# Xiaohao-Liu/EliMRec

Hardware: AMD Instinct MI355X
Metric: BPR triplets/sec (Tiktok-shape, d=128x3) (higher is better)
Workload: dtype f32; 1 GPU; tiktok-shape-synthetic; num_items=76085, train_interactions=571503, recdim=64, layer_num=3, batch_per_gpu=2048, global_batch=2048, parallelism=colshard1, graph_table=column-sharded (64 of 64 columns per rank): hops need no communication, feature_tables=replicated S_m / c, feature_dtype=f32, columns_per_gpu=64, propagation=folded, head_rows=batch, step_issue=one host call per step (csrc/program.hip): 1243 of the 1243 timed steps

## Files before the change

elimrec_amd/_lib.py:

```python
import ctypes
import os

_HERE = os.path.dirname(os.path.abspath(__file__))
LIB_PATH = os.path.join(_HERE, "lib", "libelimrec_hip.so")

c_i32, c_i64, c_f32, c_u32, c_u64 = ctypes.c_int, ctypes.c_int64, ctypes.c_float, ctypes.c_uint32, ctypes.c_uint64
c_ptr, c_size = ctypes.c_void_p, ctypes.c_size_t

class CsrSplit(ctypes.Structure):
    _fields_ = [("long_threshold", ctypes.c_int32), ("n_long", ctypes.c_int32), ("n_seg", ctypes.c_int32),
                ("d_long_rows", ctypes.c_void_p), ("d_long_seg_ptr", ctypes.c_void_p),
                ("d_seg_bounds", ctypes.c_void_p), ("d_partials", ctypes.c_void_p), ("d_seg_row", ctypes.c_void_p),
                ("d_row_order", ctypes.c_void_p), ("d_tickets", ctypes.c_void_p), ("d_row_items", ctypes.c_void_p),
                ("n_row_items", ctypes.c_int32)]


class CsrDesc(ctypes.Structure):
    _fields_ = [("n_rows", ctypes.c_int64), ("d_rowptr", ctypes.c_void_p), ("d_col", ctypes.c_void_p),
                ("d_val", ctypes.c_void_p), ("split", CsrSplit)]


class LinearDesc(ctypes.Structure):
    _fields_ = [("d_A", ctypes.c_void_p), ("lda", ctypes.c_int64), ("d_W", ctypes.c_void_p), ("ldw", ctypes.c_int64),
                ("d_bias", ctypes.c_void_p), ("d_C", ctypes.c_void_p), ("ldc", ctypes.c_int64), ("M", ctypes.c_int64),
# ... 144 lines not shown
                                 c_ptr]),
    "elimrec_topk_reference_order": (c_i32, [c_ptr, c_i64, c_i64, c_i64, c_i32, c_ptr]),
    "elimrec_topk_reference_order_device": (c_i32, [c_ptr, c_i64, c_i64, c_i64, c_i32, c_ptr, c_ptr, c_ptr]),
    "elimrec_score_topk_ordered": (c_i32, [c_ptr, c_i64, c_i64, c_i64, c_ptr, c_i32, c_i32, c_i32, c_u32, c_i32, c_i32,
                                           c_ptr, c_ptr, c_ptr, c_ptr, c_i64, c_i32, c_ptr, c_ptr, c_ptr, c_size, c_i32, c_ptr]),
    "elimrec_plan_workspace": (c_size, [c_i64, c_i64, c_i64]),
    "elimrec_plan_tile_count": (c_i64, [c_i64, c_i64, c_i64, c_i64, c_i32]),
    "elimrec_plan_rows": (c_i32, [c_ptr, c_i64, c_i32, c_i32, c_i32, c_i32, c_i32, c_i64, c_i64, c_ptr, c_ptr, c_ptr, c_ptr, c_ptr, c_ptr, c_size, c_ptr]),
    "elimrec_plan_tiles": (c_i32, [c_ptr, c_i64, c_i32, c_i32, c_i32, c_i32, c_i32, c_i64, c_i64, c_ptr, c_ptr, c_ptr, c_i64, c_i64, c_i64, c_i64, c_i64,
                                   c_i64, c_ptr, c_ptr, c_ptr, c_ptr, c_ptr, c_ptr, c_ptr, c_ptr, c_size, c_ptr]),
    "elimrec_plan_scatter": (c_i32, [c_i64, c_i32, c_ptr, c_ptr, c_ptr, c_ptr, c_ptr, c_ptr, c_ptr, c_ptr, c_ptr]),
    "elimrec_slab_sweep_lds_rows": (c_size, [c_i32]),
    "elimrec_slab_sweep_hop": (c_i32, [c_ptr, c_ptr, c_i64, c_i64, c_ptr, c_i32, c_i32, c_i32, c_i32, c_i32, c_i32,
                                       c_ptr, c_ptr, c_ptr, c_ptr, c_f32, c_ptr]),
    "elimrec_slab_sweep_hop_adam": (c_i32, [c_ptr, c_ptr, c_i64, c_i64, c_ptr, c_i32, c_i32, c_i32, c_i32, c_i32, c_i32,
                                            c_ptr, c_ptr, c_ptr, c_ptr, c_f32, c_ptr, c_ptr, c_ptr, c_ptr, c_f32, c_f32, c_f32, c_f32, c_f32,
                                            c_i64, c_ptr]),
    "elimrec_slab_hop_bwd_w": (c_i32, [c_sell, c_i32, c_i32, c_i32, c_ptr, c_ptr, c_ptr, c_ptr, c_ptr, c_f32, c_ptr, c_size, c_i32,
                                       ctypes.POINTER(LinearBwdDesc), c_i32, c_ptr, c_size, c_i32, c_ptr]),
    "elimrec_slab_source_bits": (c_i32, [c_sell, c_i32, c_i32, c_i32, c_ptr, c_ptr, c_size, c_ptr]),
    "elimrec_slab_hop_adam": (c_i32, [c_sell, c_i32, c_i32, c_i32, c_ptr, c_ptr, c_ptr, c_ptr, c_f32, c_ptr, c_size, c_ptr, c_ptr,
                                      c_ptr, c_ptr, c_f32, c_f32, c_f32, c_f32, c_f32, c_i64, ctypes.POINTER(AdamJob), c_i32, c_ptr, c_i64,
                                      c_ptr, c_ptr]),
    "elimrec_slab_rows": (c_i32, [c_sell, c_i32, c_i32, c_i32, c_i64, ctypes.POINTER(c_ptr), c_ptr, c_ptr, c_ptr, c_i64, c_i32,
                                  c_ptr, c_i64, c_ptr, c_i64, c_i32, c_ptr]),
    "elimrec_slab_from_rows": (c_i32, [c_ptr, c_i64, c_i64, c_i64, c_i32, c_i32, c_ptr, c_ptr]),
    "elimrec_slab_to_rows": (c_i32, [c_ptr, c_i64, c_i32, c_i32, c_ptr, c_i64, c_i64, c_ptr]),
    "elimrec_slab_merge_rows": (c_i32, [c_ptr, c_ptr, c_i32, c_i64, c_i64, c_i64, c_i32, c_i32, c_i32, c_ptr, c_ptr, c_ptr, c_ptr]),
    "elimrec_adam_step_out": (c_i32, [c_ptr, c_ptr, c_ptr, c_ptr, c_ptr, c_i64, c_f32, c_f32, c_f32, c_f32, c_f32, c_i64,
                                      c_ptr]),
    "elimrec_head_pack_floats": (c_size, [c_i32, ctypes.POINTER(c_i32)]),
    "elimrec_head_pack_bwd_offset": (c_size, [c_i32, ctypes.POINTER(c_i32)]),
    "elimrec_head_fwd_fused": (c_i32, [c_ptr, c_ptr, c_i64, c_ptr, c_i64, c_ptr, c_i64, c_ptr, c_i32, ctypes.POINTER(c_ptr),
                                       ctypes.POINTER(c_i64), ctypes.POINTER(c_i32), ctypes.POINTER(c_ptr), ctypes.POINTER(c_ptr),
                                       c_ptr, c_ptr, c_ptr, c_ptr, ctypes.POINTER(c_ptr), ctypes.POINTER(c_ptr), c_ptr, c_size,
                                       c_ptr, c_i64, c_ptr, c_i64, c_i32, c_i32, c_ptr]),
    "elimrec_head_fwd_fused_peers": (c_i32, [c_ptr, c_ptr, c_i64, c_ptr, c_i32, c_i64, c_ptr, c_i32, ctypes.POINTER(c_ptr),
                                             ctypes.POINTER(c_i64), ctypes.POINTER(c_i32), ctypes.POINTER(c_ptr), ctypes.POINTER(c_ptr),
                                             c_ptr, c_ptr, c_ptr, c_ptr, ctypes.POINTER(c_ptr), ctypes.POINTER(c_ptr), c_ptr, c_size,
                                             c_ptr, c_i64, c_ptr, c_i64, c_i32, c_i32, c_ptr]),
    "elimrec_head_fwd_fused_rows": (c_i32, [ctypes.POINTER(HeadRows), c_ptr, c_ptr, c_i64, c_ptr, c_i32, ctypes.POINTER(c_ptr),
                                            ctypes.POINTER(c_i64), ctypes.POINTER(c_i32), ctypes.POINTER(c_ptr), ctypes.POINTER(c_ptr),
                                            c_ptr, c_ptr, c_ptr, c_ptr, ctypes.POINTER(c_ptr), ctypes.POINTER(c_ptr), c_ptr, c_size,
                                            c_ptr, c_i64, c_ptr, c_i64, c_i32, c_ptr]),
    "elimrec_head_fwd_fused_src16": (c_i32, [ctypes.POINTER(HeadSrc16), c_ptr, c_ptr, c_i64, c_ptr, c_i64, c_ptr, c_i64, c_i32,
                                             ctypes.POINTER(c_i32), ctypes.POINTER(c_ptr), ctypes.POINTER(c_ptr), c_ptr, c_ptr, c_ptr, c_ptr,
# ... 114 lines not shown
```

elimrec_amd/csrc/program.hip:

```cpp
#include "common.h"
#include <dlfcn.h>
#include <cstring>
#include <string>
#include <utility>
#include <vector>

namespace elimrec {

template <typename T> struct Unpack {
    static T get(uint64_t v) {
        if constexpr (std::is_pointer<T>::value) return reinterpret_cast<T>(static_cast<uintptr_t>(v));
        else if constexpr (std::is_same<T, float>::value) { uint32_t b = (uint32_t)v; float f; memcpy(&f, &b, 4); return f; }
        else return static_cast<T>(v);
    }
};
template <typename R, typename... A, size_t... I>
static R call_packed_impl(R (*f)(A...), const uint64_t *a, std::index_sequence<I...>) { return f(Unpack<A>::get(a[I])...); }
template <typename R, typename... A> static R call_packed(R (*f)(A...), const uint64_t *a) {
    static_assert(sizeof...(A) <= ELIMREC_PROGRAM_MAX_ARGS, "too many arguments for a program op");
    return call_packed_impl(f, a, std::index_sequence_for<A...>{});
}
template <typename R, typename... A> constexpr int arg_count(R (*)(A...)) { return (int)sizeof...(A); }

static unsigned event_flags(bool has_collectives) {
    return has_collectives ? hipEventDisableTiming : (hipEventDisableTiming | hipEventDisableSystemFence);
}

struct FnEntry { const char *name; int (*thunk)(const uint64_t *); int n_args; };
#define ELIMREC_FN(fn) {#fn, [](const uint64_t *a) -> int { return call_packed(fn, a); }, arg_count(fn)}
static const FnEntry kFns[] = {
    ELIMREC_FN(elimrec_batch_plan), ELIMREC_FN(elimrec_slab_hop), ELIMREC_FN(elimrec_slab_sweep_hop), ELIMREC_FN(elimrec_slab_sweep_hop_adam), ELIMREC_FN(elimrec_slab_source_bits), ELIMREC_FN(elimrec_slab_hop_bwd_w),
    ELIMREC_FN(elimrec_slab_hop_adam), ELIMREC_FN(elimrec_slab_rows), ELIMREC_FN(elimrec_slab_merge_rows),
    ELIMREC_FN(elimrec_head_fwd_fused), ELIMREC_FN(elimrec_bpr_head_rows),
    ELIMREC_FN(elimrec_bpr_head_rows_sum), ELIMREC_FN(elimrec_bpr_head_rows_sum_pub), ELIMREC_FN(elimrec_sum), ELIMREC_FN(elimrec_segment_apply_head_bwd),
    ELIMREC_FN(elimrec_segment_apply_head_bwd_packed), ELIMREC_FN(elimrec_segment_apply_head_bwd_sources),
    ELIMREC_FN(elimrec_segment_apply_head_bwd_split), ELIMREC_FN(elimrec_linear_fwd_batched), ELIMREC_FN(elimrec_linear_bwd_w_batched),
    ELIMREC_FN(elimrec_linear_bwd_w_batched_merge), ELIMREC_FN(elimrec_linear_bwd_w_reduce), ELIMREC_FN(elimrec_adam_multi),
    ELIMREC_FN(elimrec_source_rows_split), ELIMREC_FN(elimrec_copy_cols), ELIMREC_FN(elimrec_lookup_pack), ELIMREC_FN(elimrec_lookup_unpack),
    ELIMREC_FN(elimrec_lookup_counts), ELIMREC_FN(elimrec_adam_step_out),
    ELIMREC_FN(elimrec_peer_cols_to_rows), ELIMREC_FN(elimrec_rows_bitmap), ELIMREC_FN(elimrec_comm_all_gather), ELIMREC_FN(elimrec_comm_all_reduce_f32),
    ELIMREC_FN(elimrec_comm_all_to_all), ELIMREC_FN(elimrec_comm_all_to_all_v), ELIMREC_FN(elimrec_wide_from_master),
    ELIMREC_FN(elimrec_wide_rows), ELIMREC_FN(elimrec_wide_grad), ELIMREC_FN(elimrec_head_fwd_fused_rows), ELIMREC_FN(elimrec_head_fwd_fused_src16),
    ELIMREC_FN(elimrec_head_fwd_fused_peers),
};
constexpr int kNumFns = (int)(sizeof(kFns) / sizeof(kFns[0]));

typedef struct ncclComm *ncclComm_t;
struct NcclId { char internal[128]; };
struct Rccl {
    void *h = nullptr;
    int (*GetUniqueId)(NcclId *) = nullptr;
    int (*CommInitRank)(ncclComm_t *, int, NcclId, int) = nullptr;
    int (*CommDestroy)(ncclComm_t) = nullptr;
    int (*CommCount)(ncclComm_t, int *) = nullptr;
    int (*AllGather)(const void *, void *, size_t, int, ncclComm_t, hipStream_t) = nullptr;
// ... 185 lines not shown
```

elimrec_amd/csrc/slab.hip:

```cpp
#include "common.h"
#include "merge_rows.h"
#include "rows_args.h"
#include "bwd_w.h"
#include <cstdlib>

namespace elimrec {


struct SellArgs {
    const int32_t *item_dst, *item_len, *blk_off, *col;
    const float *val;
    int64_t n_rows, n_src;
    int n_seg, n_long;
    int item_begin, item_end;
    int seg_limit;
    int w4, w4_shift, gs, spg;
    const float4 *Xin;
    const uint32_t *src_mask;
    float4 *Xout;
    const float4 *Add;
    const uint32_t *add_mask;
    float scale;
    float4 *partials;
    const int32_t *long_rows, *long_seg_ptr;
// ... 329 lines not shown
    int64_t n;
    float step_size, inv_sqrt_bc2;
    int first_block;
};
struct AdamJobs {
    AdamJob j[8]; int n; int blocks;
    const float *sum_src; float *sum_dst; int sum_n;
};

__device__ __forceinline__ void fixed_order_sum_body(const float *__restrict__ x, int n, float *__restrict__ out, float *s) {
    for (int vt = threadIdx.x; vt < 1024; vt += 256) {
        float acc = 0.f;
        for (int i = vt; i < n; i += 1024) acc += x[i];
        s[vt] = acc;
    }
    __syncthreads();
    for (int w = 512; w > 0; w >>= 1) {
        for (int idx = threadIdx.x; idx < w; idx += 256) s[idx] += s[idx + w];
        __syncthreads();
    }
    if (threadIdx.x == 0) out[0] = s[0];
}

__device__ __forceinline__ void adam_jobs_body(const AdamJobs &jobs, int block, float beta1, float beta2, float eps, float wd) {
    int k = 0;
    while (k + 1 < jobs.n && block >= jobs.j[k + 1].first_block) ++k;
    const AdamJob &jb = jobs.j[k];
    const int nb = (k + 1 < jobs.n ? jobs.j[k + 1].first_block : jobs.blocks) - jb.first_block;
    for (int64_t i = (int64_t)(block - jb.first_block) * 256 + threadIdx.x; i < jb.n; i += (int64_t)nb * 256) {
        const float pi = jb.p_in[i];
        if (jb.copy_dst) jb.copy_dst[i] = pi;
        if (!jb.g) continue;
        const float gi = fmaf(wd, pi, jb.g[i]);
        const float mi = jb.m[i] + (1.f - beta1) * (gi - jb.m[i]);
        const float vi = fmaf(1.f - beta2, gi * gi, beta2 * jb.v[i]);
        const float denom = sqrtf(vi) * jb.inv_sqrt_bc2 + eps;
        jb.m[i] = mi;
        jb.v[i] = vi;
        const float po = pi - jb.step_size * (mi / denom);
        jb.p_out[i] = po;
    }
}

__global__ __launch_bounds__(256) void adam_multi_kernel(AdamJobs jobs, float beta1, float beta2, float eps, float wd) {
    adam_jobs_body(jobs, (int)blockIdx.x, beta1, beta2, eps, wd);
}

struct TierArgs {
    StreamArgs s;
    const int64_t *tile_off;
    const int32_t *tile_len, *tile_dst, *tile_long, *tcol, *long_index;
    const float *tval;
    int n_w4;
    int t1_base, tseg_base, tfin_base, n_tiles;
    int n_tiles_run;
    const uint64_t *ballots;
// ... 243 lines not shown
    }
}

#ifndef ELIMREC_TILE_WAVES
#define ELIMREC_TILE_WAVES 5
#endif
template <int LPR, int VPL, bool IN_BF16, bool OUT_BF16, bool MASKED>
__global__ __launch_bounds__(256, ELIMREC_TILE_WAVES) void sell_tier_kernel(TierArgs t) {
    tier_body<LPR, VPL, IN_BF16, OUT_BF16, MASKED, false>(t);
}

template <int LPR>
__global__ __launch_bounds__(256) void sell_tier_adam_kernel(TierArgs t, AdamJobs tail, int tail_block0) {
    __shared__ float scratch[4 * 64 * 8];
    if ((int)blockIdx.x >= tail_block0) {
        const int b = (int)blockIdx.x - tail_block0;
        if (b < tail.blocks) adam_jobs_body(tail, b, t.s.ad_beta1, t.s.ad_beta2, t.s.ad_eps, t.s.ad_wd);
        else fixed_order_sum_body(tail.sum_src, tail.sum_n, tail.sum_dst, scratch);
        return;
    }
    tier_body<LPR, 4, false, false, false, true, true>(t, scratch);
}

template <int LPR, bool MASKED>
__global__ __launch_bounds__(256, (LPR <= 8 ? 5 : 1)) void sell_tier_bwdw_kernel(TierArgs t, BwdBatch batch, int tail_block0, int tail_mode, int gx) {
    __shared__ float As[2][TRB * TN1];
    __shared__ float Bs[2][TRB * TN2];
    static_assert(2 * TRB * TN1 >= 4 * 64 * 8, "the hop's LDS scratch must fit the A stages");
    const int front = tail_block0 < 0 ? (-tail_block0 + 7) & ~7 : 0;
    if (tail_block0 < 0 ? (int)blockIdx.x < front : (int)blockIdx.x >= tail_block0) {
        const int b = tail_block0 < 0 ? (int)blockIdx.x : (int)blockIdx.x - tail_block0;
        if (tail_block0 < 0 && b >= -tail_block0) return;
        if (tail_mode == 1) { reduce_slabs_body(batch, b % gx, b / gx); return; }
        bwd_w_partial_body(batch, b, As, Bs);
        return;
    }
    tier_body<LPR, 4, false, false, MASKED, false, true>(t, &As[0][0], (unsigned)front);
}

static int log2_pow2(int x) {
    int s = 0;
    while ((1 << s) < x) ++s;
    return (1 << s) == x ? s : -1;
}

}

using namespace elimrec;

static size_t slab_partial_floats_bytes(const elimrec_sell *A, int ns, int w) {
    return align_up((size_t)(A->n_seg > 0 ? A->n_seg : 1) * ns * w * sizeof(float), 256);
}
static size_t slab_ticket_bytes(const elimrec_sell *A) { return align_up((size_t)8 * (A->n_long > 0 ? A->n_long : 1) * sizeof(int32_t), 256); }
static size_t slab_ballot_bytes(const elimrec_sell *A) {
    if (!A->tiered) return 0;
    const size_t tiles = (size_t)A->n_t4 + A->n_t1 + A->n_tseg + A->n_tfin;
    return align_up(tiles * (size_t)(A->tile_kmax > 0 ? A->tile_kmax : 1) * sizeof(uint64_t), 256);
}

extern "C" size_t elimrec_slab_partials_bytes(const elimrec_sell *A, int ns, int w) {
    if (!A || ns <= 0 || w <= 0) return 0;
    return slab_partial_floats_bytes(A, ns, w) + slab_ticket_bytes(A) + slab_ballot_bytes(A);
}

struct AdamEpilogue {
    const float *p_in; float *p_out, *m, *v;
    float step_size, inv_sqrt_bc2, beta1, beta2, eps, wd;
    int keep_grad;
    const AdamJobs *tail;
};

static int launch_tier(const elimrec_sell *A, int ns, int wl, int wl_shift, int gs, int spg, int lpr, const void *Xin,
                       const uint32_t *src_mask, void *Xout, const float *add,
                       const uint32_t *add_mask, float scale, float *partials, int flags, hipStream_t s,
                       const AdamEpilogue *adam = nullptr, const BwdBatch *bwdw = nullptr, int tail_mode = 0, int tail_blocks = 0,
                       int reduce_gx = 1) {
    const int seg_only = flags & 1;
    const bool bits_ready = (flags & 2) != 0;
    if (A->tile_groups != 64 / lpr) {
        set_error("slab_hop: the plan's wave tiles were laid out for %d lane groups per wave, this table geometry has %d",
                  A->tile_groups, 64 / lpr);
        return ELIMREC_E_BADARG;
    }
    ELIMREC_REQUIRE(A->d_tile_off && A->d_tile_len && A->d_tile_dst && A->d_tile_col && A->d_tile_val && A->n_t4 == 4 * A->n_w4 &&
                        A->n_t1 % 4 == 0 && A->n_tseg % 4 == 0 && A->n_tfin % 4 == 0 && (A->n_tseg == 0 || A->d_tile_long),
                    "slab_hop: bad tile plan");
    TierArgs t = {};
    StreamArgs &a = t.s;
    a.n_rows = A->n_rows; a.n_src = A->n_src; a.n_seg = A->n_seg; a.n_long = A->n_long;
    a.wl = wl; a.wl_shift = wl_shift; a.gs = gs; a.spg = spg;
    a.Xin = Xin; a.src_mask = src_mask; a.Xout = Xout;
    a.Add = seg_only ? nullptr : (const float4 *)add; a.add_mask = add_mask; a.scale = seg_only ? 1.0f : scale;
// ... 16 lines not shown
    int tail_block0 = (int)(per_group * gs);
    {
        if (bwdw && tail_blocks > 0 && !adam && tail_mode == 2) {
            tail_block0 = -tail_blocks;
            tail_blocks = (tail_blocks + 7) & ~7;
        }
    }
    AdamJobs tail = {};
    if (adam && adam->tail && (adam->tail->n > 0 || adam->tail->sum_src)) tail = *adam->tail;
    if (tail.n <= 0) tail.blocks = 0;
    const dim3 grid((unsigned)(per_group * gs)), grid_adam((unsigned)(per_group * gs) + (unsigned)tail.blocks + (tail.sum_src ? 1u : 0u));
    const bool masked = src_mask != nullptr;
    if (masked) {
        ELIMREC_REQUIRE(A->tile_kmax > 0, "slab_hop: bad tile plan (tile_kmax)");
        t.kmax = A->tile_kmax;
        uint64_t *ballots = (uint64_t *)((char *)a.tickets + slab_ticket_bytes(A));
        t.ballots = ballots;
        if (!bits_ready)
        hipLaunchKernelGGL(tile_ballot_kernel, dim3((unsigned)per_group, (unsigned)t.kmax), dim3(256), 0, s, t.tile_off, t.tcol, src_mask, 64 / lpr,
                           t.n_tiles_run, t.kmax, ballots);
    }
#define ELIMREC_TIER(LPR)                                                                                                     \
    do {                                                                                                                      \
        if (adam) hipLaunchKernelGGL((sell_tier_adam_kernel<LPR>), grid_adam, dim3(256), 0, s, t, tail, tail_block0);         \
        else if (bwdw && masked)                                                                                              \
            hipLaunchKernelGGL((sell_tier_bwdw_kernel<LPR, true>), dim3(grid.x + (unsigned)tail_blocks), dim3(256), 0, s, t,  \
                               *bwdw, tail_block0, tail_mode, reduce_gx);                                                     \
        else if (bwdw)                                                                                                        \
            hipLaunchKernelGGL((sell_tier_bwdw_kernel<LPR, false>), dim3(grid.x + (unsigned)tail_blocks), dim3(256), 0, s, t, \
                               *bwdw, tail_block0, tail_mode, reduce_gx);                                                     \
        else if (masked) hipLaunchKernelGGL((sell_tier_kernel<LPR, 4, false, false, true>), grid, dim3(256), 0, s, t);        \
        else hipLaunchKernelGGL((sell_tier_kernel<LPR, 4, false, false, false>), grid, dim3(256), 0, s, t);                   \
    } while (0)
    switch (lpr) {
        case 1: ELIMREC_TIER(1); break;
        case 2: ELIMREC_TIER(2); break;
        case 4: ELIMREC_TIER(4); break;
        case 8: ELIMREC_TIER(8); break;
        case 16: ELIMREC_TIER(16); break;
        case 32: ELIMREC_TIER(32); break;
        default: ELIMREC_TIER(64); break;
    }
#undef ELIMREC_TIER
    return check_hip(hipGetLastError(), "slab_hop(tiered)");
}

static int slab_geometry(const char *who, int ns, int w, int gs, int &w4_shift, int &spg, int &lpr) {
// ... 127 lines not shown
extern "C" int elimrec_slab_hop_bwd_w(const elimrec_sell *A, int ns, int w, int gs, const float *d_Xin, const uint32_t *d_src_mask,
                                      float *d_Xout, const float *d_add, const uint32_t *d_add_mask, float scale, float *d_partials,
                                      size_t partials_bytes, int flags, const elimrec_linear_bwd_desc *descs, int n,
                                      void *d_workspace, size_t workspace_bytes, int phase, void *stream) {
    ELIMREC_REQUIRE(A && d_Xin && d_Xout && d_Xin != d_Xout, "slab_hop_bwd_w: null pointer / alias");
    ELIMREC_REQUIRE(A->tiered && !(flags & 1), "slab_hop_bwd_w: needs a tiered (wave-tile) plan and a full hop");
    ELIMREC_REQUIRE(phase == 0 || phase == 1, "slab_hop_bwd_w: phase 0 (partial launch) or 1 (slab reduce)");
    ELIMREC_REQUIRE(descs && n >= 1 && n <= kMaxBatch, "slab_hop_bwd_w: 1..%d problems", kMaxBatch);
    ELIMREC_REQUIRE(d_workspace && workspace_bytes >= bwd_w_batched_bytes(descs, n), "slab_hop_bwd_w: weight-gradient workspace");
    int w4_shift, spg, lpr, rc;
    if ((rc = slab_geometry("slab_hop_bwd_w", ns, w, gs, w4_shift, spg, lpr))) return rc;
    if (!d_partials || partials_bytes < elimrec_slab_partials_bytes(A, ns, w)) {
        set_error("slab_hop_bwd_w: partial-row scratch too small");
        return ELIMREC_E_WORKSPACE;
    }
    BwdBatch batch;
    int blocks = 0, max_out = 0;
    if ((rc = bwd_w_build_batch(descs, n, d_workspace, batch, blocks, max_out))) return rc;
    const int gx = (4 * max_out + 255) / 256;
    return launch_tier(A, ns, w / 4, w4_shift, gs, spg, lpr, d_Xin, d_src_mask, d_Xout, d_add, d_add_mask, scale,
                       d_partials, flags, (hipStream_t)stream, nullptr, &batch, phase == 0 ? 2 : 1, phase == 0 ? blocks : gx * n, gx);
}

extern "C" int elimrec_slab_hop_adam(const elimrec_sell *A, int ns, int w, int gs, const float *d_Xin, float *d_grad_out,
                                     const float *d_add, const uint32_t *d_add_mask, float scale, float *d_partials,
                                     size_t partials_bytes, const float *d_p_in, float *d_p_out, float *d_m, float *d_v, float lr,
                                     float beta1, float beta2, float eps, float weight_decay, int64_t step,
                                     const elimrec_adam_job *tail_jobs, int n_tail_jobs, const float *d_sum_src, int64_t sum_n,
                                     float *d_sum_dst, void *stream) {
    ELIMREC_REQUIRE(A && d_Xin && d_p_in && d_p_out && d_m && d_v, "slab_hop_adam: null pointer");
    ELIMREC_REQUIRE(!d_sum_src || (d_sum_dst && sum_n >= 0 && sum_n < INT32_MAX), "slab_hop_adam: the sum needs a destination");
    ELIMREC_REQUIRE(A->tiered, "slab_hop_adam: needs a tiered (wave-tile) plan");
    ELIMREC_REQUIRE(step >= 1, "slab_hop_adam: 1-based step");
    ELIMREC_REQUIRE((const void *)d_Xin != (const void *)d_p_out && (const void *)d_Xin != (const void *)d_m &&
                        (const void *)d_Xin != (const void *)d_v, "slab_hop_adam: the gathered table must not be written");
    int w4_shift, spg, lpr, rc;
    if ((rc = slab_geometry("slab_hop_adam", ns, w, gs, w4_shift, spg, lpr))) return rc;
    if (!d_partials || partials_bytes < elimrec_slab_partials_bytes(A, ns, w)) {
        set_error("slab_hop_adam: partial-row scratch too small");
        return ELIMREC_E_WORKSPACE;
    }
    AdamEpilogue ad;
    ad.p_in = d_p_in; ad.p_out = d_p_out; ad.m = d_m; ad.v = d_v;
    const double bc1 = 1.0 - pow((double)beta1, (double)step), bc2 = 1.0 - pow((double)beta2, (double)step);
    ad.step_size = (float)((double)lr / bc1);
    ad.inv_sqrt_bc2 = (float)(1.0 / sqrt(bc2));
    ad.beta1 = beta1; ad.beta2 = beta2; ad.eps = eps; ad.wd = weight_decay; ad.keep_grad = d_grad_out ? 1 : 0;
    AdamJobs tail = {};
    ad.tail = nullptr;
    if (tail_jobs && n_tail_jobs > 0) {
        ELIMREC_REQUIRE(n_tail_jobs <= 8, "slab_hop_adam: at most 8 tail jobs");
        if ((rc = build_adam_jobs("slab_hop_adam", tail_jobs, n_tail_jobs, lr, beta1, beta2, tail))) return rc;
        ad.tail = &tail;
    }
    if (d_sum_src) { tail.sum_src = d_sum_src; tail.sum_dst = d_sum_dst; tail.sum_n = (int)sum_n; ad.tail = &tail; }
    return launch_tier(A, ns, w / 4, w4_shift, gs, spg, lpr, d_Xin, nullptr, d_grad_out, d_add, d_add_mask, scale,
                       d_partials, 0, (hipStream_t)stream, &ad);
}

extern "C" int elimrec_slab_rows(const elimrec_sell *A, int ns, int w, int L, int64_t U, const float *const *layers,
                                 const float *d_long, const int32_t *d_rows, const int32_t *d_counts, int64_t R,
                                 int n_lists, float *d_out0, int64_t ld_out0, float *d_narrow, int64_t ld_narrow,
                                 int narrow_by_node, void *stream) {
    ELIMREC_REQUIRE(A && layers && d_out0 && d_narrow, "slab_rows: null pointer");
    ELIMREC_REQUIRE(ld_out0 % 4 == 0 && ld_narrow % 4 == 0, "slab_rows: leading dimensions must be multiples of 4");
    ELIMREC_REQUIRE(n_lists >= 1 && (d_rows || n_lists == 1), "slab_rows: several lists need row ids");
    RowsArgs a = {};
    int rc;
    if ((rc = rows_args_fill("slab_rows", A, ns, w, L, U, layers, d_long, a))) return rc;
    a.rows = d_rows; a.counts = d_counts; a.R = R; a.n_lists = n_lists;
    a.out0 = d_out0; a.ld_out0 = ld_out0; a.narrow = d_narrow; a.ld_narrow = ld_narrow; a.by_node = narrow_by_node;
    const int64_t total = R * n_lists;
    if (total <= 0) return 0;
    int lr = 1;
    while (lr < a.nc4 && lr < 64) lr *= 2;
    hipStream_t s = (hipStream_t)stream;
    const unsigned blocks = (unsigned)((total + (256 / lr) - 1) / (256 / lr));
    switch (lr) {
        case 1: hipLaunchKernelGGL((slab_rows_kernel<1>), dim3(blocks), dim3(256), 0, s, a); break;
        case 2: hipLaunchKernelGGL((slab_rows_kernel<2>), dim3(blocks), dim3(256), 0, s, a); break;
// ... 125 lines not shown
```

elimrec_amd/shard.py:

```python
import ctypes

import numpy as np
import torch
import torch.distributed as dist

from . import _lib, ops, program, slab
from .lookup import FeatureShard, RowOwnerMap

PAD_KEY = -(1 << 30)


def _all_gather_parts(loc, world, group):
    if loc.is_cuda and dist.get_backend(group) == "gloo":
        host = loc.cpu()
        parts = [torch.empty_like(host) for _ in range(world)]
        dist.all_gather(parts, host, group=group)
        return [p.to(loc.device) for p in parts]
    parts = [torch.empty_like(loc) for _ in range(world)]
    dist.all_gather(parts, loc, group=group)
    return parts


LOSS_RING = 1 << 16

# ... 1263 lines not shown
        return send, wg

    def join_source_bits(self):
        if getattr(self, "_bits_join", False):
            program.sync(torch.cuda.current_stream(), self._aux)
            self._bits_join = False

    @torch.no_grad()
    def cs_backward_hops(self, recv2, acts, grads_ready=None, reduce_wgrads=None):
        m = self.model
        U, I, L = m.num_users, m.num_items, m.n_layers
        W, R = acts.shape
        inv = 1.0 / (L + 1)

        fuse = self._fuse_adam() and not getattr(self, "grads_only", False)
        last = 1 if fuse else 0

        single = not self.multi
        merged = single and getattr(self, "_merged", False)
        self.join_source_bits()
        reduce = getattr(self, "_reduce", None) if (single or reduce_wgrads is not None) else None
        self._reduce = None
        self.wgrads_handle = None

        if self.wide:
            def wide_hops():
                slab.merge_rows(recv2.view(W * R, 2 * self.dl), acts.reshape(-1), W, U, I, self.srcA, self.srcB, self.mask, M=-1)
                t, tmask = self.srcW, self.mask
                for k in range(L - 1, -1, -1):
                    dst = self.tmp[k & 1]
                    slab.hop(self.planT, t, dst, gs=self.hgs, src_mask=tmask, add=self.srcW, add_mask=self.mask, scale=1.0,
                             bits_ready=tmask is not None and self._bits_ready)
                    t, tmask = dst, None
                slab.wide_grad(t, U, inv, self.grad)
            self._timed(lambda: m._region("cs_bwd_hops", (m._ws_gen, recv2.data_ptr(), acts.data_ptr(), R, W, self._bits_ready), wide_hops), L)
            self._adam_in_hop = self._tail_in_hop = False
            if reduce_wgrads is not None and reduce_wgrads is not True:
                self.wgrads_handle = reduce_wgrads()
            return

        def hops():
            phase = None if reduce is None else reduce[1]
            if merged:
                pass
            elif single:
                slab.merge_rows(recv2.view(R, m.C), acts.reshape(-1), 1, U, I, self.srcA, self.srcB, self.mask, M=m.M)
            else:
                slab.merge_rows(recv2.view(W * R, 2 * self.dl), acts.reshape(-1), W, U, I, self.srcA, self.srcB, self.mask)
            t, tmask = (self.srcB if (L & 1) else self.srcA), self.mask
            for k in range(L - 1, last - 1, -1):
                dst = self.grad if k == 0 else self.tmp[k & 1]
                slab.hop(self.planT, t, dst, gs=self.gs, src_mask=tmask, add=self.srcB if (k & 1) else self.srcA,
                         add_mask=self.mask, scale=inv if k == 0 else 1.0, bits_ready=tmask is not None and self._bits_ready,
                         bwd_w=reduce[0] if phase is not None and phase <= 1 else None, bwd_w_phase=phase)
                phase = None if phase is None else phase + 1
                t, tmask = dst, None
        self._timed(lambda: m._region("cs_bwd_hops", (m._ws_gen, recv2.data_ptr(), acts.data_ptr(), R, W, fuse, self._bits_ready, merged,
                                                               0 if reduce is None else ctypes.addressof(reduce[0][0]), 0 if reduce is None else reduce[1]), hops), L - last)
        self._adam_in_hop = fuse
        self._tail_in_hop = False
        if fuse:
            g = self.opt.param_groups[0]
            nxt = 1 - self.cur
            in_hop = single or grads_ready is not None
            if reduce_wgrads is True:
                in_hop = True
            elif reduce_wgrads is not None:
                self.wgrads_handle = reduce_wgrads()
                in_hop = False
            if grads_ready is not None:
                grads_ready.wait()
            tail = self._tail_jobs() if in_hop else []
            if len(tail) > 8:
                raise RuntimeError("more than 8 optimizer spans")
            if getattr(self, "_tail_arr", None) is None:
                self._tail_arr = (_lib.AdamJob * 8)()
            for i, job in enumerate(tail):
                self._tail_arr[i] = job
            self._tail_n, self._tail_base = len(tail), 0
            tail = (self._tail_arr, len(tail))
            self._tail_in_hop = in_hop
            late = getattr(self, "_loss_late", None)
            self._loss_late = None
            self._timed(lambda: slab.hop_adam(self.planT, self.tmp[1], self.grad if self.keep_grad else None, self.gs, self.srcA,
                                              self.mask, inv, self.master[self.cur].data, self.master[nxt].data, self.m1, self.m2,
                                              g["lr"], g["betas"][0], g["betas"][1], g["eps"], g["weight_decay"],
                                              self.step_count + 1, tail_jobs=tail, loss_sum=late), 1)

    @torch.no_grad()
    def cs_update(self):
        m = self.model
        g = self.opt.param_groups[0]
        self.step_count += 1
        nxt = 1 - self.cur
        jobs = []
        if not getattr(self, "_adam_in_hop", False):
            jobs.append(_lib.AdamJob(self.master[self.cur].data.data_ptr(), self.master[nxt].data.data_ptr(),
                                     self.grad.data.data_ptr(),
                                     self.m1.data_ptr(), self.m2.data_ptr(), None, self.grad.data.numel(), self.step_count))
        if not getattr(self, "_tail_in_hop", False):
            jobs += self._tail_jobs()
        if len(jobs) > 8:
            raise RuntimeError("more than 8 optimizer spans")
        if jobs:
            if getattr(self, "_tail_arr", None) is None:
                self._tail_arr = (_lib.AdamJob * 8)()
            for i, job in enumerate(jobs):
                self._tail_arr[i] = job
            self._tail_base = 0 if getattr(self, "_adam_in_hop", False) else 1
            self._tail_n = len(jobs) - self._tail_base
# ... 321 lines not shown
```

elimrec_amd/slab.py:

```python
import ctypes
import os

import numpy as np
import torch

from . import _lib
from .ops import _dev, _stream

LONG_ROW_THRESHOLD = 32
SLAB_W_CAP = 32
SLAB_GROUPS = 0


def choose_slabs(dl, n_rows=None):
    if dl % 4 != 0:
        raise ValueError("column count must be a multiple of 4 (got %d)" % dl)
    cap = SLAB_W_CAP
    w = 4
    while w * 2 <= cap and dl % (w * 2) == 0:
        w *= 2
    return dl // w, w


def choose_groups(ns):
# ... 431 lines not shown
    if _swept(plan, xin) and src_mask is None and not seg_only and isinstance(xout, SlabTable):
        hop(plan.sweep.items, xin, xout, gs=gs, add=add, add_mask=add_mask, scale=scale, bwd_w=bwd_w, bwd_w_phase=bwd_w_phase)
        plan.sweep.hop(xin, xout, add=add, add_mask=add_mask, scale=scale)
        return
    part = plan.partials(ns, w)
    out = xout if isinstance(xout, torch.Tensor) else xout.data
    lib = _lib.load()
    if bwd_w is not None:
        arr, n, wsp = bwd_w
        _lib.check(lib.elimrec_slab_hop_bwd_w(plan.ref(), ns, w, int(gs), _dev(xin.data, "xin"), _dev(src_mask, "src_mask", torch.int32),
                                               _dev(out, "xout"), _dev(None if add is None else add.data, "add"),
                                               _dev(add_mask, "add_mask", torch.int32), float(scale), _dev(part, "partials"),
                                               part.numel() * 4, 2 if bits_ready else 0, arr, n, _dev(wsp, "workspace", torch.uint8),
                                               wsp.numel(), int(bwd_w_phase), _stream()), "slab_hop_bwd_w")
        return
    _lib.check(lib.elimrec_slab_hop(plan.ref(), ns, w, int(gs), _dev(xin.data, "xin"),
                                    _dev(src_mask, "src_mask", torch.int32), _dev(out, "xout"),
                                    _dev(None if add is None else add.data, "add"),
                                    _dev(add_mask, "add_mask", torch.int32), float(scale), _dev(part, "partials"),
                                    part.numel() * 4, (1 if seg_only else 0) | (2 if bits_ready else 0), _stream()), "slab_hop")


def hop_adam(plan, xin, grad_out, gs, add, add_mask, scale, p_in, p_out, m, v, lr, beta1, beta2, eps, weight_decay, step, tail_jobs=(),
             loss_sum=None):
    if isinstance(tail_jobs, tuple) and len(tail_jobs) == 2 and not isinstance(tail_jobs[0], _lib.AdamJob):
        arr, n_tail = tail_jobs
    else:
        arr, n_tail = ((_lib.AdamJob * len(tail_jobs))(*tail_jobs) if tail_jobs else None), len(tail_jobs)
    ns, w = xin.ns, xin.w
    if _swept(plan, xin):
        hop_adam(plan.sweep.items, xin, grad_out, gs, add, add_mask, scale, p_in, p_out, m, v, lr, beta1, beta2, eps, weight_decay, step,
                 tail_jobs=(arr, n_tail), loss_sum=loss_sum)
        plan.sweep.hop_adam(xin, grad_out, add, add_mask, scale, p_in, p_out, m, v, lr, beta1, beta2, eps, weight_decay, step)
        return
    part = plan.partials(ns, w)
    _lib.check(_lib.load().elimrec_slab_hop_adam(
        plan.ref(), ns, w, int(gs), _dev(xin.data, "xin"), _dev(None if grad_out is None else grad_out.data, "grad"),
        _dev(None if add is None else add.data, "add"), _dev(add_mask, "add_mask", torch.int32), float(scale), _dev(part, "partials"),
        part.numel() * 4, _dev(p_in, "p_in"), _dev(p_out, "p_out"), _dev(m, "m"), _dev(v, "v"), float(lr), float(beta1), float(beta2),
        float(eps), float(weight_decay), int(step), arr, n_tail, _dev(None if loss_sum is None else loss_sum[0], "loss_rows"),
        0 if loss_sum is None else loss_sum[0].numel(), _dev(None if loss_sum is None else loss_sum[1], "loss_out"), _stream()),
        "slab_hop_adam")



def rows(plan, ns, w, L, U, layers, long_tab, row_ids, counts, R, n_lists, out0, narrow, narrow_by_node):
    ptrs = (ctypes.c_void_p * (L + 1))(*[None if t is None else _dev(t, "layer") for t in layers])
    assert out0.stride(1) == 1 and narrow.stride(1) == 1
    _lib.check(_lib.load().elimrec_slab_rows(plan.ref(), ns, w, L, int(U), ptrs, _dev(long_tab, "long_tab"),
                                             _dev(row_ids, "rows", torch.int32), _dev(counts, "counts", torch.int32),
                                             int(R), int(n_lists), _dev(out0, "out0"), out0.stride(0),
                                             _dev(narrow, "narrow"), narrow.stride(0), 1 if narrow_by_node else 0,
                                             _stream()), "slab_rows")


def merge_rows(all_rows, all_keys, world, U, I, srcA, srcB, mask, M=0):
    R = all_keys.numel() // world
    assert all_rows.is_contiguous() and all_rows.shape == (world * R, (M if M > 0 else 2) * srcA.cols) and mask.numel() * 32 >= U + I
    _lib.check(_lib.load().elimrec_slab_merge_rows(_dev(all_rows, "rows"), _dev(all_keys, "keys", torch.int32), int(world), R,
                                                   int(U), int(I), srcA.ns, srcA.w, int(M), _dev(srcA.data, "srcA"),
                                                   _dev(srcB.data, "srcB"), _dev(mask, "mask", torch.int32), _stream()),
               "slab_merge_rows")


def adam_step_out(p_in, p_out, g, m, v, lr, beta1, beta2, eps, weight_decay, step):
# ... 34 lines not shown
```

include/elimrec_hip.h:

```cpp
#ifndef ELIMREC_HIP_H
#define ELIMREC_HIP_H

#include <stddef.h>
#include <stdint.h>

#ifdef __cplusplus
extern "C" {
#endif

#define ELIMREC_ABI_VERSION 1
#define ELIMREC_E_BADARG 10001
#define ELIMREC_E_UNSUPPORTED 10002
#define ELIMREC_E_WORKSPACE 10003

int elimrec_abi_version(void);
const char *elimrec_last_error(void);

int elimrec_linear_fwd(const float *d_A, int64_t lda, const float *d_W, int64_t ldw,
                       const float *d_bias, float *d_C, int64_t ldc,
                       int64_t M, int N, int K, void *stream);

typedef struct elimrec_linear_desc {
    const float *d_A; int64_t lda;
    const float *d_W; int64_t ldw;
// ... 305 lines not shown
                           int max_block_rows, int ns, int w, const float *d_Xin, float *d_Xout,
                           const float *d_add, const uint32_t *d_add_mask, float scale, void *stream);
int elimrec_slab_sweep_hop_adam(const int64_t *d_slot_ptr, const void *d_records, int64_t n_rows, int64_t n_src,
                                const int32_t *d_block_ptr, int parts, int passes, int bpx, int max_block_rows, int ns, int w,
                                const float *d_Xin, float *d_grad_out, const float *d_add, const uint32_t *d_add_mask, float scale,
                                const float *d_p_in, float *d_p_out, float *d_m, float *d_v, float lr, float beta1, float beta2,
                                float eps, float weight_decay, int64_t step , void *stream);

int elimrec_slab_source_bits(const elimrec_sell *A, int ns, int w, int gs, const uint32_t *d_src_mask,
                             float *d_partials, size_t partials_bytes, void *stream);

int elimrec_slab_hop_bwd_w(const elimrec_sell *A, int ns, int w, int gs, const float *d_Xin, const uint32_t *d_src_mask,
                           float *d_Xout, const float *d_add, const uint32_t *d_add_mask, float scale, float *d_partials,
                           size_t partials_bytes, int flags, const elimrec_linear_bwd_desc *descs , int n,
                           void *d_workspace, size_t workspace_bytes, int phase, void *stream);

struct elimrec_adam_job;
int elimrec_slab_hop_adam(const elimrec_sell *A, int ns, int w, int gs, const float *d_Xin, float *d_grad_out,
                          const float *d_add, const uint32_t *d_add_mask, float scale, float *d_partials,
                          size_t partials_bytes, const float *d_p_in, float *d_p_out, float *d_m, float *d_v, float lr,
                          float beta1, float beta2, float eps, float weight_decay, int64_t step,
                          const struct elimrec_adam_job *tail_jobs, int n_tail_jobs, const float *d_sum_src, int64_t sum_n,
                          float *d_sum_dst, void *stream);

int elimrec_slab_rows(const elimrec_sell *A, int ns, int w, int L, int64_t U,
                      const float *const *layers, const float *d_long, const int32_t *d_rows,
                      const int32_t *d_counts, int64_t R, int n_lists, float *d_out0, int64_t ld_out0,
                      float *d_narrow, int64_t ld_narrow, int narrow_by_node, void *stream);

int elimrec_slab_from_rows(const float *d_src, int64_t ld, int64_t col0, int64_t n, int ns, int w,
                           float *d_slab, void *stream);
int elimrec_slab_to_rows(const float *d_slab, int64_t n, int ns, int w, float *d_dst, int64_t ld,
                         int64_t col0, void *stream);

int elimrec_slab_merge_rows(const float *d_rows, const int32_t *d_keys, int world, int64_t R, int64_t U,
                            int64_t I, int ns, int w, int M, float *d_SrcA, float *d_SrcB, uint32_t *d_mask,
                            void *stream);

int elimrec_adam_step_out(const float *d_p_in, float *d_p_out, const float *d_g, float *d_m, float *d_v,
                          int64_t n, float lr, float beta1, float beta2, float eps, float weight_decay,
                          int64_t step, void *stream);

size_t elimrec_head_pack_floats(int n_mod, const int *D);
size_t elimrec_head_pack_bwd_offset(int n_mod, const int *D);
int elimrec_head_fwd_fused(const int32_t *d_act, const int32_t *d_seg_info, int64_t R, const float *d_out0,
                           int64_t ld_out0, const float *d_narrow, int64_t ld_nar, const float *d_c, int n_mod,
// ... 103 lines not shown
```

Baseline: 7.282 million triplets/s.

## Fold weight-gradient slab reduce into the fused hop-Adam tail optimizer

```diff
diff --git a/elimrec_amd/_lib.py b/elimrec_amd/_lib.py
--- a/elimrec_amd/_lib.py
+++ b/elimrec_amd/_lib.py
@@ -190,6 +190,9 @@
     "elimrec_slab_hop_adam": (c_i32, [c_sell, c_i32, c_i32, c_i32, c_ptr, c_ptr, c_ptr, c_ptr, c_f32, c_ptr, c_size, c_ptr, c_ptr,
                                       c_ptr, c_ptr, c_f32, c_f32, c_f32, c_f32, c_f32, c_i64, ctypes.POINTER(AdamJob), c_i32, c_ptr, c_i64,
                                       c_ptr, c_ptr]),
+    "elimrec_slab_hop_adam_wgrad": (c_i32, [c_sell, c_i32, c_i32, c_i32, c_ptr, c_ptr, c_ptr, c_ptr, c_f32, c_ptr, c_size, c_ptr, c_ptr,
+                                            c_ptr, c_ptr, c_f32, c_f32, c_f32, c_f32, c_f32, c_i64, ctypes.POINTER(AdamJob), c_i32, c_ptr,
+                                            c_i64, c_ptr, ctypes.POINTER(LinearBwdDesc), c_i32, c_ptr, c_size, c_ptr]),
     "elimrec_slab_rows": (c_i32, [c_sell, c_i32, c_i32, c_i32, c_i64, ctypes.POINTER(c_ptr), c_ptr, c_ptr, c_ptr, c_i64, c_i32,
                                   c_ptr, c_i64, c_ptr, c_i64, c_i32, c_ptr]),
     "elimrec_slab_from_rows": (c_i32, [c_ptr, c_i64, c_i64, c_i64, c_i32, c_i32, c_ptr, c_ptr]),
diff --git a/elimrec_amd/csrc/program.hip b/elimrec_amd/csrc/program.hip
--- a/elimrec_amd/csrc/program.hip
+++ b/elimrec_amd/csrc/program.hip
@@ -30,7 +30,7 @@
 #define ELIMREC_FN(fn) {#fn, [](const uint64_t *a) -> int { return call_packed(fn, a); }, arg_count(fn)}
 static const FnEntry kFns[] = {
     ELIMREC_FN(elimrec_batch_plan), ELIMREC_FN(elimrec_slab_hop), ELIMREC_FN(elimrec_slab_sweep_hop), ELIMREC_FN(elimrec_slab_sweep_hop_adam), ELIMREC_FN(elimrec_slab_source_bits), ELIMREC_FN(elimrec_slab_hop_bwd_w),
-    ELIMREC_FN(elimrec_slab_hop_adam), ELIMREC_FN(elimrec_slab_rows), ELIMREC_FN(elimrec_slab_merge_rows),
+    ELIMREC_FN(elimrec_slab_hop_adam), ELIMREC_FN(elimrec_slab_hop_adam_wgrad), ELIMREC_FN(elimrec_slab_rows), ELIMREC_FN(elimrec_slab_merge_rows),
     ELIMREC_FN(elimrec_head_fwd_fused), ELIMREC_FN(elimrec_bpr_head_rows),
     ELIMREC_FN(elimrec_bpr_head_rows_sum), ELIMREC_FN(elimrec_bpr_head_rows_sum_pub), ELIMREC_FN(elimrec_sum), ELIMREC_FN(elimrec_segment_apply_head_bwd),
     ELIMREC_FN(elimrec_segment_apply_head_bwd_packed), ELIMREC_FN(elimrec_segment_apply_head_bwd_sources),
diff --git a/elimrec_amd/csrc/slab.hip b/elimrec_amd/csrc/slab.hip
--- a/elimrec_amd/csrc/slab.hip
+++ b/elimrec_amd/csrc/slab.hip
@@ -375,7 +375,60 @@
     if (threadIdx.x == 0) out[0] = s[0];
 }
 
-__device__ __forceinline__ void adam_jobs_body(const AdamJobs &jobs, int block, float beta1, float beta2, float eps, float wd) {
+struct SlabGrad {
+    const float *out, *colsum;
+    const float *slabs, *cslabs;
+    const int32_t *range;
+    int64_t R, ldo, out_span;
+    int n1, n2, n1_pad, n2_pad, chunk_rows;
+};
+struct SlabGrads { SlabGrad p[kMaxBatch]; int n; };
+
+__device__ __forceinline__ bool slab_grad(const SlabGrads &sg, const float *addr, float &g) {
+    const float *src = nullptr;
+    size_t stride = 0;
+    int chunks = 0;
+    for (int k = 0; k < sg.n && !src; ++k) {
+        const SlabGrad &p = sg.p[k];
+        const int64_t off = ((int64_t)(uintptr_t)addr - (int64_t)(uintptr_t)p.out) >> 2;
+        if (off >= 0 && off < p.out_span) {
+            const int64_t i = off / p.ldo, j = off - i * p.ldo;
+            if (j < p.n2) {
+                src = p.slabs + (size_t)i * p.n2_pad + j;
+                stride = (size_t)p.n1_pad * p.n2_pad;
+            }
+        } else if (p.colsum) {
+            const int64_t offc = ((int64_t)(uintptr_t)addr - (int64_t)(uintptr_t)p.colsum) >> 2;
+            if (offc >= 0 && offc < p.n1) {
+                src = p.cslabs + offc;
+                stride = (size_t)p.n1_pad;
+            }
+        }
+        if (src) {
+            int64_t rows = p.range ? (int64_t)p.range[1] - p.range[0] : p.R;
+            if (rows < 0) rows = 0;
+            chunks = (int)((rows + p.chunk_rows - 1) / p.chunk_rows);
+        }
+    }
+    if (!src) return false;
+    float s0 = 0.f, s1 = 0.f, s2 = 0.f, s3 = 0.f;
+    int c = 0;
+#pragma unroll 4
+    for (; c + 4 <= chunks; c += 4) {
+        const float v0 = src[(size_t)c * stride], v1 = src[(size_t)(c + 1) * stride];
+        const float v2 = src[(size_t)(c + 2) * stride], v3 = src[(size_t)(c + 3) * stride];
+        s0 += v0; s1 += v1; s2 += v2; s3 += v3;
+    }
+    if (c < chunks) s0 += src[(size_t)c * stride];
+    if (c + 1 < chunks) s1 += src[(size_t)(c + 1) * stride];
+    if (c + 2 < chunks) s2 += src[(size_t)(c + 2) * stride];
+    g = (s0 + s1) + (s2 + s3);
+    return true;
+}
+
+template <bool SLABS = false>
+__device__ __forceinline__ void adam_jobs_body(const AdamJobs &jobs, int block, float beta1, float beta2, float eps, float wd,
+                                               const SlabGrads *sg = nullptr) {
     int k = 0;
     while (k + 1 < jobs.n && block >= jobs.j[k + 1].first_block) ++k;
     const AdamJob &jb = jobs.j[k];
@@ -384,7 +437,9 @@
         const float pi = jb.p_in[i];
         if (jb.copy_dst) jb.copy_dst[i] = pi;
         if (!jb.g) continue;
-        const float gi = fmaf(wd, pi, jb.g[i]);
+        float graw;
+        if (!(SLABS && slab_grad(*sg, jb.g + i, graw))) graw = jb.g[i];
+        const float gi = fmaf(wd, pi, graw);
         const float mi = jb.m[i] + (1.f - beta1) * (gi - jb.m[i]);
         const float vi = fmaf(1.f - beta2, gi * gi, beta2 * jb.v[i]);
         const float denom = sqrtf(vi) * jb.inv_sqrt_bc2 + eps;
@@ -674,6 +729,18 @@
     tier_body<LPR, 4, false, false, false, true, true>(t, scratch);
 }
 
+template <int LPR>
+__global__ __launch_bounds__(256) void sell_tier_adam_wgrad_kernel(TierArgs t, AdamJobs tail, SlabGrads sg, int tail_block0) {
+    __shared__ float scratch[4 * 64 * 8];
+    if ((int)blockIdx.x >= tail_block0) {
+        const int b = (int)blockIdx.x - tail_block0;
+        if (b < tail.blocks) adam_jobs_body<true>(tail, b, t.s.ad_beta1, t.s.ad_beta2, t.s.ad_eps, t.s.ad_wd, &sg);
+        else fixed_order_sum_body(tail.sum_src, tail.sum_n, tail.sum_dst, scratch);
+        return;
+    }
+    tier_body<LPR, 4, false, false, false, true, true>(t, scratch);
+}
+
 template <int LPR, bool MASKED>
 __global__ __launch_bounds__(256, (LPR <= 8 ? 5 : 1)) void sell_tier_bwdw_kernel(TierArgs t, BwdBatch batch, int tail_block0, int tail_mode, int gx) {
     __shared__ float As[2][TRB * TN1];
@@ -720,6 +787,7 @@
     float step_size, inv_sqrt_bc2, beta1, beta2, eps, wd;
     int keep_grad;
     const AdamJobs *tail;
+    const SlabGrads *wgrad;
 };
 
 static int launch_tier(const elimrec_sell *A, int ns, int wl, int wl_shift, int gs, int spg, int lpr, const void *Xin,
@@ -782,7 +850,9 @@
     }
 #define ELIMREC_TIER(LPR)                                                                                                     \
     do {                                                                                                                      \
-        if (adam) hipLaunchKernelGGL((sell_tier_adam_kernel<LPR>), grid_adam, dim3(256), 0, s, t, tail, tail_block0);         \
+        if (adam && adam->wgrad)                                                                                              \
+            hipLaunchKernelGGL((sell_tier_adam_wgrad_kernel<LPR>), grid_adam, dim3(256), 0, s, t, tail, *adam->wgrad, tail_block0); \
+        else if (adam) hipLaunchKernelGGL((sell_tier_adam_kernel<LPR>), grid_adam, dim3(256), 0, s, t, tail, tail_block0);    \
         else if (bwdw && masked)                                                                                              \
             hipLaunchKernelGGL((sell_tier_bwdw_kernel<LPR, true>), dim3(grid.x + (unsigned)tail_blocks), dim3(256), 0, s, t,  \
                                *bwdw, tail_block0, tail_mode, reduce_gx);                                                     \
@@ -956,12 +1026,13 @@
                        d_partials, flags, (hipStream_t)stream, nullptr, &batch, phase == 0 ? 2 : 1, phase == 0 ? blocks : gx * n, gx);
 }
 
-extern "C" int elimrec_slab_hop_adam(const elimrec_sell *A, int ns, int w, int gs, const float *d_Xin, float *d_grad_out,
-                                     const float *d_add, const uint32_t *d_add_mask, float scale, float *d_partials,
-                                     size_t partials_bytes, const float *d_p_in, float *d_p_out, float *d_m, float *d_v, float lr,
-                                     float beta1, float beta2, float eps, float weight_decay, int64_t step,
-                                     const elimrec_adam_job *tail_jobs, int n_tail_jobs, const float *d_sum_src, int64_t sum_n,
-                                     float *d_sum_dst, void *stream) {
+static int slab_hop_adam(const elimrec_sell *A, int ns, int w, int gs, const float *d_Xin, float *d_grad_out,
+                         const float *d_add, const uint32_t *d_add_mask, float scale, float *d_partials,
+                         size_t partials_bytes, const float *d_p_in, float *d_p_out, float *d_m, float *d_v, float lr,
+                         float beta1, float beta2, float eps, float weight_decay, int64_t step,
+                         const elimrec_adam_job *tail_jobs, int n_tail_jobs, const float *d_sum_src, int64_t sum_n,
+                         float *d_sum_dst, const elimrec_linear_bwd_desc *descs, int n_descs, void *d_workspace,
+                         size_t workspace_bytes, void *stream) {
     ELIMREC_REQUIRE(A && d_Xin && d_p_in && d_p_out && d_m && d_v, "slab_hop_adam: null pointer");
     ELIMREC_REQUIRE(!d_sum_src || (d_sum_dst && sum_n >= 0 && sum_n < INT32_MAX), "slab_hop_adam: the sum needs a destination");
     ELIMREC_REQUIRE(A->tiered, "slab_hop_adam: needs a tiered (wave-tile) plan");
@@ -982,6 +1053,27 @@
     ad.beta1 = beta1; ad.beta2 = beta2; ad.eps = eps; ad.wd = weight_decay; ad.keep_grad = d_grad_out ? 1 : 0;
     AdamJobs tail = {};
     ad.tail = nullptr;
+    ad.wgrad = nullptr;
+    SlabGrads sg = {};
+    if (descs) {
+        ELIMREC_REQUIRE(n_descs >= 1 && n_descs <= kMaxBatch, "slab_hop_adam_wgrad: 1..%d problems", kMaxBatch);
+        ELIMREC_REQUIRE(tail_jobs && n_tail_jobs > 0, "slab_hop_adam_wgrad: no optimizer span to consume the weight gradients");
+        ELIMREC_REQUIRE(d_workspace && workspace_bytes >= bwd_w_batched_bytes(descs, n_descs), "slab_hop_adam_wgrad: weight-gradient workspace");
+        BwdBatch batch;
+        int blocks = 0, max_out = 0;
+        if ((rc = bwd_w_build_batch(descs, n_descs, d_workspace, batch, blocks, max_out))) return rc;
+        sg.n = n_descs;
+        for (int i = 0; i < n_descs; ++i) {
+            const BwdProblem &pb = batch.p[i];
+            ELIMREC_REQUIRE(!pb.d.accumulate, "slab_hop_adam_wgrad: problem %d accumulates into its output (run the reduce instead)", i);
+            ELIMREC_REQUIRE(pb.d.ldo >= pb.d.n2, "slab_hop_adam_wgrad: problem %d: ldo < n2", i);
+            SlabGrad &o = sg.p[i];
+            o.out = pb.d.d_out; o.colsum = pb.d.d_colsum; o.slabs = pb.slabs; o.cslabs = pb.cslabs; o.range = pb.d.d_range;
+            o.R = pb.d.R; o.ldo = pb.d.ldo; o.out_span = (int64_t)(pb.d.n1 - 1) * pb.d.ldo + pb.d.n2;
+            o.n1 = pb.d.n1; o.n2 = pb.d.n2; o.n1_pad = pb.t1 * TN1; o.n2_pad = pb.t2 * TN2; o.chunk_rows = pb.chunk_rows;
+        }
+        ad.wgrad = &sg;
+    }
     if (tail_jobs && n_tail_jobs > 0) {
         ELIMREC_REQUIRE(n_tail_jobs <= 8, "slab_hop_adam: at most 8 tail jobs");
         if ((rc = build_adam_jobs("slab_hop_adam", tail_jobs, n_tail_jobs, lr, beta1, beta2, tail))) return rc;
@@ -990,6 +1082,30 @@
     if (d_sum_src) { tail.sum_src = d_sum_src; tail.sum_dst = d_sum_dst; tail.sum_n = (int)sum_n; ad.tail = &tail; }
     return launch_tier(A, ns, w / 4, w4_shift, gs, spg, lpr, d_Xin, nullptr, d_grad_out, d_add, d_add_mask, scale,
                        d_partials, 0, (hipStream_t)stream, &ad);
+}
+
+extern "C" int elimrec_slab_hop_adam(const elimrec_sell *A, int ns, int w, int gs, const float *d_Xin, float *d_grad_out,
+                                     const float *d_add, const uint32_t *d_add_mask, float scale, float *d_partials,
+                                     size_t partials_bytes, const float *d_p_in, float *d_p_out, float *d_m, float *d_v, float lr,
+                                     float beta1, float beta2, float eps, float weight_decay, int64_t step,
+                                     const elimrec_adam_job *tail_jobs, int n_tail_jobs, const float *d_sum_src, int64_t sum_n,
+                                     float *d_sum_dst, void *stream) {
+    return slab_hop_adam(A, ns, w, gs, d_Xin, d_grad_out, d_add, d_add_mask, scale, d_partials, partials_bytes, d_p_in, d_p_out, d_m,
+                         d_v, lr, beta1, beta2, eps, weight_decay, step, tail_jobs, n_tail_jobs, d_sum_src, sum_n, d_sum_dst, nullptr, 0,
+                         nullptr, 0, stream);
+}
+
+extern "C" int elimrec_slab_hop_adam_wgrad(const elimrec_sell *A, int ns, int w, int gs, const float *d_Xin, float *d_grad_out,
+                                           const float *d_add, const uint32_t *d_add_mask, float scale, float *d_partials,
+                                           size_t partials_bytes, const float *d_p_in, float *d_p_out, float *d_m, float *d_v, float lr,
+                                           float beta1, float beta2, float eps, float weight_decay, int64_t step,
+                                           const elimrec_adam_job *tail_jobs, int n_tail_jobs, const float *d_sum_src, int64_t sum_n,
+                                           float *d_sum_dst, const elimrec_linear_bwd_desc *descs, int n_descs, void *d_workspace,
+                                           size_t workspace_bytes, void *stream) {
+    ELIMREC_REQUIRE(descs, "slab_hop_adam_wgrad: null problem table");
+    return slab_hop_adam(A, ns, w, gs, d_Xin, d_grad_out, d_add, d_add_mask, scale, d_partials, partials_bytes, d_p_in, d_p_out, d_m,
+                         d_v, lr, beta1, beta2, eps, weight_decay, step, tail_jobs, n_tail_jobs, d_sum_src, sum_n, d_sum_dst, descs,
+                         n_descs, d_workspace, workspace_bytes, stream);
 }
 
 extern "C" int elimrec_slab_rows(const elimrec_sell *A, int ns, int w, int L, int64_t U, const float *const *layers,
diff --git a/elimrec_amd/shard.py b/elimrec_amd/shard.py
--- a/elimrec_amd/shard.py
+++ b/elimrec_amd/shard.py
@@ -1309,6 +1309,7 @@
         reduce = getattr(self, "_reduce", None) if (single or reduce_wgrads is not None) else None
         self._reduce = None
         self.wgrads_handle = None
+        fold = (fuse and single and reduce is not None and not self.keep_grad and not self.word_train)
 
         if self.wide:
             def wide_hops():
@@ -1339,11 +1340,12 @@
                 dst = self.grad if k == 0 else self.tmp[k & 1]
                 slab.hop(self.planT, t, dst, gs=self.gs, src_mask=tmask, add=self.srcB if (k & 1) else self.srcA,
                          add_mask=self.mask, scale=inv if k == 0 else 1.0, bits_ready=tmask is not None and self._bits_ready,
-                         bwd_w=reduce[0] if phase is not None and phase <= 1 else None, bwd_w_phase=phase)
+                         bwd_w=reduce[0] if phase is not None and phase <= (0 if fold else 1) else None, bwd_w_phase=phase)
                 phase = None if phase is None else phase + 1
                 t, tmask = dst, None
         self._timed(lambda: m._region("cs_bwd_hops", (m._ws_gen, recv2.data_ptr(), acts.data_ptr(), R, W, fuse, self._bits_ready, merged,
-                                                               0 if reduce is None else ctypes.addressof(reduce[0][0]), 0 if reduce is None else reduce[1]), hops), L - last)
+                                                               0 if reduce is None else ctypes.addressof(reduce[0][0]), 0 if reduce is None else reduce[1],
+                                                               fold), hops), L - last)
         self._adam_in_hop = fuse
         self._tail_in_hop = False
         if fuse:
@@ -1365,6 +1367,8 @@
             for i, job in enumerate(tail):
                 self._tail_arr[i] = job
             self._tail_n, self._tail_base = len(tail), 0
+            if fold and not tail:
+                raise RuntimeError("the weight gradients' slab reduce was left to the optimizer spans, and there is none")
             tail = (self._tail_arr, len(tail))
             self._tail_in_hop = in_hop
             late = getattr(self, "_loss_late", None)
@@ -1372,7 +1376,8 @@
             self._timed(lambda: slab.hop_adam(self.planT, self.tmp[1], self.grad if self.keep_grad else None, self.gs, self.srcA,
                                               self.mask, inv, self.master[self.cur].data, self.master[nxt].data, self.m1, self.m2,
                                               g["lr"], g["betas"][0], g["betas"][1], g["eps"], g["weight_decay"],
-                                              self.step_count + 1, tail_jobs=tail, loss_sum=late), 1)
+                                              self.step_count + 1, tail_jobs=tail, loss_sum=late,
+                                              wgrad=reduce[0] if fold else None), 1)
 
     @torch.no_grad()
     def cs_update(self):
diff --git a/elimrec_amd/slab.py b/elimrec_amd/slab.py
--- a/elimrec_amd/slab.py
+++ b/elimrec_amd/slab.py
@@ -477,25 +477,30 @@
 
 
 def hop_adam(plan, xin, grad_out, gs, add, add_mask, scale, p_in, p_out, m, v, lr, beta1, beta2, eps, weight_decay, step, tail_jobs=(),
-             loss_sum=None):
+             loss_sum=None, wgrad=None):
     if isinstance(tail_jobs, tuple) and len(tail_jobs) == 2 and not isinstance(tail_jobs[0], _lib.AdamJob):
         arr, n_tail = tail_jobs
     else:
         arr, n_tail = ((_lib.AdamJob * len(tail_jobs))(*tail_jobs) if tail_jobs else None), len(tail_jobs)
     ns, w = xin.ns, xin.w
     if _swept(plan, xin):
+        assert wgrad is None, "the swept form keeps the weight gradients' slab reduce as a launch"
         hop_adam(plan.sweep.items, xin, grad_out, gs, add, add_mask, scale, p_in, p_out, m, v, lr, beta1, beta2, eps, weight_decay, step,
                  tail_jobs=(arr, n_tail), loss_sum=loss_sum)
         plan.sweep.hop_adam(xin, grad_out, add, add_mask, scale, p_in, p_out, m, v, lr, beta1, beta2, eps, weight_decay, step)
         return
     part = plan.partials(ns, w)
-    _lib.check(_lib.load().elimrec_slab_hop_adam(
-        plan.ref(), ns, w, int(gs), _dev(xin.data, "xin"), _dev(None if grad_out is None else grad_out.data, "grad"),
-        _dev(None if add is None else add.data, "add"), _dev(add_mask, "add_mask", torch.int32), float(scale), _dev(part, "partials"),
-        part.numel() * 4, _dev(p_in, "p_in"), _dev(p_out, "p_out"), _dev(m, "m"), _dev(v, "v"), float(lr), float(beta1), float(beta2),
-        float(eps), float(weight_decay), int(step), arr, n_tail, _dev(None if loss_sum is None else loss_sum[0], "loss_rows"),
-        0 if loss_sum is None else loss_sum[0].numel(), _dev(None if loss_sum is None else loss_sum[1], "loss_out"), _stream()),
-        "slab_hop_adam")
+    args = (plan.ref(), ns, w, int(gs), _dev(xin.data, "xin"), _dev(None if grad_out is None else grad_out.data, "grad"),
+            _dev(None if add is None else add.data, "add"), _dev(add_mask, "add_mask", torch.int32), float(scale), _dev(part, "partials"),
+            part.numel() * 4, _dev(p_in, "p_in"), _dev(p_out, "p_out"), _dev(m, "m"), _dev(v, "v"), float(lr), float(beta1), float(beta2),
+            float(eps), float(weight_decay), int(step), arr, n_tail, _dev(None if loss_sum is None else loss_sum[0], "loss_rows"),
+            0 if loss_sum is None else loss_sum[0].numel(), _dev(None if loss_sum is None else loss_sum[1], "loss_out"))
+    if wgrad is not None:
+        descs, n, wsp = wgrad
+        _lib.check(_lib.load().elimrec_slab_hop_adam_wgrad(*args, descs, n, _dev(wsp, "workspace", torch.uint8), wsp.numel(), _stream()),
+                   "slab_hop_adam_wgrad")
+        return
+    _lib.check(_lib.load().elimrec_slab_hop_adam(*args, _stream()), "slab_hop_adam")
 
 
 
diff --git a/include/elimrec_hip.h b/include/elimrec_hip.h
--- a/include/elimrec_hip.h
+++ b/include/elimrec_hip.h
@@ -351,6 +351,13 @@
                           float beta1, float beta2, float eps, float weight_decay, int64_t step,
                           const struct elimrec_adam_job *tail_jobs, int n_tail_jobs, const float *d_sum_src, int64_t sum_n,
                           float *d_sum_dst, void *stream);
+int elimrec_slab_hop_adam_wgrad(const elimrec_sell *A, int ns, int w, int gs, const float *d_Xin, float *d_grad_out,
+                                const float *d_add, const uint32_t *d_add_mask, float scale, float *d_partials,
+                                size_t partials_bytes, const float *d_p_in, float *d_p_out, float *d_m, float *d_v, float lr,
+                                float beta1, float beta2, float eps, float weight_decay, int64_t step,
+                                const struct elimrec_adam_job *tail_jobs, int n_tail_jobs, const float *d_sum_src, int64_t sum_n,
+                                float *d_sum_dst, const elimrec_linear_bwd_desc *descs , int n_descs,
+                                void *d_workspace, size_t workspace_bytes, void *stream);
 
 int elimrec_slab_rows(const elimrec_sell *A, int ns, int w, int L, int64_t U,
                       const float *const *layers, const float *d_long, const int32_t *d_rows,
```

Measured after the change: 7.472 million triplets/s (median of 6 runs). +2.6%, better.
